# SHI-Labs/Self-Similarity-Grouping

Measured on AMD Instinct MI355X. Metric: images/s embed + s/iter for NxN rerank+DBSCAN, N=16k, 1/2/4/8 GPU, higher is better.
Workload: dtype f32 (embed: split-half operands hi+lo on fp16 MFMA, fp32 accumulate, 6e-8 max error vs the fp32 reference features) / exact int64 via int8 MFMA digits + f64 + f16 (distance, re-rank: half semantics, bit-exact)

## Files before the change

include/ssg_hip.h:

```cpp
#ifndef SSG_HIP_H
#define SSG_HIP_H

#include <stddef.h>
#include <stdint.h>

#ifdef __cplusplus
extern "C" {
#endif

typedef struct ihipStream_t* ssg_stream_t;

#define SSG_OK 0
#define SSG_ERR_INVALID (-1)
#define SSG_ERR_HIP (-2)
#define SSG_ERR_OVERFLOW (-3)
#define SSG_ERR_NAN (-4)

const char* ssg_last_error(void);
int ssg_version(void);
uint16_t ssg_double_to_half_bits(double d);

int ssg_range_stats_f32(const float* a, int rows_a, const float* b, int rows_b, int d, float* out4, ssg_stream_t stream);
int ssg_row_norms_f64(const float* x, int n, int d, int round_to_half, double* norms, ssg_stream_t stream);
int ssg_sqdist_self_f16(const float* x, const double* norms, int N, int d, int row0, int nrows, int memory_save, uint16_t* D, uint32_t* rowmax,
// ... 96 lines not shown
                      void* ws, size_t ws_bytes, int64_t* labels, ssg_stream_t stream);

int ssg_conv2d_nhwc_f32(const float* in, const float* w, const float* bias, const float* res, float* out, int B, int H, int W, int Cin,
                        int Cout, int KH, int KW, int stride, int pad, int relu, ssg_stream_t stream);
int ssg_conv1x1_dual_nhwc_f32(const float* in, const float* in2, const float* w, const float* bias, float* out, int B, int H, int W, int Cin,
                              int H2, int W2, int Cin2, int stride2, int Cout, int relu, ssg_stream_t stream);
#define SSG_CONV_IN_SPLIT 1
#define SSG_CONV_OUT_SPLIT 2
int ssg_conv2d_nhwc_x(const void* in, const void* w, const float* bias, const void* res, void* out, int B, int H, int W, int Cin,
                      int Cout, int KH, int KW, int stride, int pad, int relu, int flags, float acc_scale, const float* ch_scale,
                      int32_t* overflow, ssg_stream_t stream);
int ssg_conv1x1_dual_nhwc_x(const void* in, const void* in2, const void* w, const float* bias, void* out, int B, int H, int W, int Cin,
                            int H2, int W2, int Cin2, int stride2, int Cout, int relu, int flags, float acc_scale, const float* ch_scale,
                            int32_t* overflow, ssg_stream_t stream);
#define SSG_CONV_W_TILED 4
int ssg_conv_weights_tile_supported(int Cout, int Kpad);
int ssg_conv_weights_tile(const void* w, int Cout, int Kpad, void* wt, ssg_stream_t stream);
int ssg_conv2d_nhwc_xt(const void* in, const void* w, const void* wt, const float* bias, const void* res, void* out, int B, int H, int W, int Cin,
                       int Cout, int KH, int KW, int stride, int pad, int relu, int flags, float acc_scale, const float* ch_scale,
                       int32_t* overflow, ssg_stream_t stream);
int ssg_conv1x1_dual_nhwc_xt(const void* in, const void* in2, const void* w, const void* wt, const float* bias, void* out, int B, int H, int W, int Cin,
                             int H2, int W2, int Cin2, int stride2, int Cout, int relu, int flags, float acc_scale, const float* ch_scale,
                             int32_t* overflow, ssg_stream_t stream);
int ssg_conv_pair_supported(int K1, int C, int N2);
int ssg_conv_pair_nhwc_x(const void* y2, const void* w3, const float* b3, const float* cs3, const void* res, void* out,
                         const void* w1n, const float* b1n, const float* cs1n, void* y1n, int M, int K1, int C, int N2,
                         int32_t* overflow, ssg_stream_t stream);
int ssg_bottleneck_supported(int H, int W, int CIN, int C, int MID);
int ssg_bottleneck_nhwc_x(const void* x, const void* w1, const float* b1, const float* cs1, const void* w2, const float* b2, const float* cs2,
                          const void* w3, const float* b3, const float* cs3, void* out, int B, int H, int W, int C, int MID,
                          int32_t* overflow, ssg_stream_t stream);
int ssg_bottleneck_ds_nhwc_x(const void* x, const void* w1, const float* b1, const float* cs1, const void* w2, const float* b2, const float* cs2,
                             const void* w3cat, const float* b3, const float* cs3, void* out, int B, int H, int W, int CIN, int C, int MID,
                             int32_t* overflow, ssg_stream_t stream);
int ssg_basicblock_supported(int H, int W, int C);
int ssg_basicblock_nhwc_x(const void* x, const void* w1, const float* b1, const float* cs1, const void* w2, const float* b2, const float* cs2,
                          void* out, int B, int H, int W, int C, int32_t* overflow, ssg_stream_t stream);
int ssg_stem_pool_supported(int H, int W);
int ssg_stem_pool_nchw_x(const float* images, int flip, const void* w, const float* bias, const float* ch_scale, void* out, int B, int H, int W,
                         int32_t* overflow, ssg_stream_t stream);
int ssg_nchw_to_nhwc4_h4l4(const float* in, void* out, int B, int H, int W, int flip, ssg_stream_t stream);
int ssg_maxpool3x3s2_h8l8(const void* in, void* out, int B, int H, int W, int C, ssg_stream_t stream);
int ssg_gap_stripes_h8l8(const void* in, float* out, int B, int H, int W, int C, int num_split, ssg_stream_t stream);
int ssg_h8l8_encode(const float* in, void* out, int64_t n, float scale, ssg_stream_t stream);
int ssg_h8l8_decode(const void* in, float* out, int64_t n, float scale, ssg_stream_t stream);
int ssg_pairwise_sqdist_f32(const float* x, const float* y, int m, int n, int d, int self_form, float* ws, float* out, ssg_stream_t stream);
// ... 186 lines not shown
```

self-similarity-grouping_amd/csrc/conv.hip:

```cpp
#include "ssg_common.h"
#include <cstdlib>
#include <type_traits>

namespace ssg {

typedef float v16f __attribute__((ext_vector_type(16)));
typedef unsigned int v4u __attribute__((ext_vector_type(4)));
typedef _Float16 v8h __attribute__((ext_vector_type(8)));

__device__ __forceinline__ unsigned pack_h2(_Float16 a, _Float16 b) {
  return (unsigned)__builtin_bit_cast(unsigned short, a) | ((unsigned)__builtin_bit_cast(unsigned short, b) << 16);
}
__device__ __forceinline__ float unpack_lo(unsigned u) { return (float)__builtin_bit_cast(_Float16, (unsigned short)(u & 0xffffu)); }
__device__ __forceinline__ float unpack_hi(unsigned u) { return (float)__builtin_bit_cast(_Float16, (unsigned short)(u >> 16)); }
__device__ __forceinline__ void split_encode4(const float4 v, uint2& hi, uint2& lo) {
  const _Float16 h0 = (_Float16)v.x, h1 = (_Float16)v.y, h2 = (_Float16)v.z, h3 = (_Float16)v.w;
  hi = make_uint2(pack_h2(h0, h1), pack_h2(h2, h3));
  lo = make_uint2(pack_h2((_Float16)(v.x - (float)h0), (_Float16)(v.y - (float)h1)), pack_h2((_Float16)(v.z - (float)h2), (_Float16)(v.w - (float)h3)));
}
__device__ __forceinline__ bool split_hi_nonfinite(const uint2 hi) {
  const unsigned a = hi.x & 0x7fff7fffu, b = hi.y & 0x7fff7fffu;
  return (a & 0xffffu) >= 0x7c00u || (a >> 16) >= 0x7c00u || (b & 0xffffu) >= 0x7c00u || (b >> 16) >= 0x7c00u;
}
__device__ __forceinline__ float4 split_decode4(const uint2 hi, const uint2 lo) {
  return make_float4(unpack_lo(hi.x) + unpack_lo(lo.x), unpack_hi(hi.x) + unpack_hi(lo.x), unpack_lo(hi.y) + unpack_lo(lo.y), unpack_hi(hi.y) + unpack_hi(lo.y));
}

struct ConvParams {
  const float* in; const float* w; const float* bias; const float* res = nullptr; float* out;
  int B, H, W, Cin, OH, OW, Cout, KH, KW, stride, pad, relu;
  int M, Kpad;
  unsigned in_bytes;
  const float* in2 = nullptr; int H2 = 0, W2 = 0, Cin2 = 0, stride2 = 1, nk1; unsigned in2_bytes = 0;
  const float* rowterm = nullptr; int epi = 0;
  float* tilemin = nullptr; int tmin_ld = 0;
  int out_split = 0, res_split = 0; float acc_scale = 1.f;
  const float* cscale = nullptr;
  int* overflow = nullptr;
  const float* wt = nullptr;
  unsigned long long* prof = nullptr;
};
#ifdef SSG_DMA_PROF
#define SSG_DMA_STAMP(I_) { if (p.prof && threadIdx.x == 0) p.prof[(size_t)blockIdx.x * 8 + (I_)] = __builtin_readcyclecounter(); }
#else
#define SSG_DMA_STAMP(I_)
#endif

constexpr int CLD32 = 36;

__device__ __forceinline__ int conv_xcd_remap(int b, int nwg) {
  const int nx = 8, q = nwg / nx, r = nwg % nx, x = b % nx, s = b / nx;
  return (x < r ? x * (q + 1) : r * (q + 1) + (x - r) * q) + s;
}

template <int MT, int NT> struct SplitFrags { v8h ah[MT], al[MT], bh[NT], bl[NT]; };

typedef float v4f __attribute__((ext_vector_type(4)));
template <int MT, int NT, int CLD, bool TAP4>
__device__ __forceinline__ void split_load_frags(const float* Arow, const float* Brow, const int kofs, SplitFrags<MT, NT>& f) {
#pragma unroll
  for (int i = 0; i < MT; i++) {
    const float* q = Arow + i * 32 * CLD + kofs;
    if (TAP4) {
// ... 360 lines not shown
          v.x += r4.x; v.y += r4.y; v.z += r4.z; v.w += r4.w;
        }
        if (p.relu) { v.x = v.x > 0.f ? v.x : 0.f; v.y = v.y > 0.f ? v.y : 0.f; v.z = v.z > 0.f ? v.z : 0.f; v.w = v.w > 0.f ? v.w : 0.f; }
        if (p.out_split) {
          uint2 hp, lp;
          split_encode4(v, hp, lp);
          if (p.overflow && split_hi_nonfinite(hp)) *p.overflow = 1;
          const uint2 send = h ? hp : lp;
          const uint2 recv = make_uint2((unsigned)__shfl_xor((int)send.x, 32, 64), (unsigned)__shfl_xor((int)send.y, 32, 64));
          const uint4 st = h ? make_uint4(recv.x, recv.y, lp.x, lp.y) : make_uint4(hp.x, hp.y, recv.x, recv.y);
#ifdef SSG_IGEMM_NT_STORE
          if (m < p.M) { const v4u sv_ = {st.x, st.y, st.z, st.w}; __builtin_nontemporal_store(sv_, reinterpret_cast<v4u*>(outp + (int64_t)m * p.Cout + col)); }
#else
          if (m < p.M) *reinterpret_cast<uint4*>(outp + (int64_t)m * p.Cout + col) = st;
#endif
        } else if (m < p.M) *reinterpret_cast<float4*>(outp + (int64_t)m * p.Cout + col) = v;
      }
    }
  }
}

#define SSG_LDSP(ptr_) ((__attribute__((address_space(3))) void*)(ptr_))

template <int BM, int BN, bool DUAL = false, int LINE = 0>
__global__ __launch_bounds__((BM / 64) * (BN / 64) * 64, BM == 256 ? 1 : (BN == 256 ? 4 : 3)) void conv_dma_kernel(ConvParams p) {
  static_assert((BM == 128 && (BN == 128 || BN == 256)) || (BM == 256 && BN == 256), "128 x 128, 128 x 256 or 256 x 256 tiles");
  static_assert(LINE == 0 || LINE == 1, "k-tile order or line order");
  constexpr int NS = BM == 256 ? 4 : 3;
  constexpr int WM = 64, WN = 64, MT = WM / 32, NT = 2, CBK = 16;
  constexpr int WCOLS = BN / WN, NW = (BM / WM) * WCOLS;
  constexpr int ABLK = BM / 16 / NW, WBLK = BN / 16 / NW;
  constexpr int STAGE_BYTES = (BM + BN) * 64;
  __shared__ __attribute__((aligned(1024))) unsigned char st0[STAGE_BYTES];
  __shared__ __attribute__((aligned(1024))) unsigned char st1[STAGE_BYTES];
  __shared__ __attribute__((aligned(1024))) unsigned char st2[STAGE_BYTES];
  __shared__ __attribute__((aligned(1024))) unsigned char st3[NS == 4 ? STAGE_BYTES : 1024];
  const int tiles_n = p.Cout / BN, tiles_m = (p.M + BM - 1) / BM;
  const int tile = conv_xcd_remap((int)blockIdx.x, tiles_m * tiles_n);
  const int tm = tile / tiles_n, tn = tile % tiles_n;
  const int tid = (int)threadIdx.x, lane = tid & 63, wave = __builtin_amdgcn_readfirstlane(tid >> 6);
  SSG_DMA_STAMP(0)
  const int wm = wave / WCOLS, wn = wave % WCOLS, l32 = lane & 31, h = lane >> 5;

  const int drow = lane >> 2, pc = lane & 3;
  const int lc4 = (pc ^ ((drow >> 2) & 3)) * 4;
  const int nkA = DUAL ? p.nk1 * 2 : 0x7fffffff;
  int ab0, ah0, aw0, ab1 = -1, ah1 = 0, aw1 = 0, abase0 = 0, abase1 = 0;
  unsigned a2b0 = 0x80000000u, a2b1 = 0x80000000u;
#define SSG_ROW(J)                                                                                                   \
  {                                                                                                                  \
// ... 166 lines not shown
    if constexpr (NS == 4) { if (nk - nfull == 3) { asm volatile("s_waitcnt vmcnt(0) lgkmcnt(0)\n\ts_barrier" ::: "memory"); SSG_LAST(st2) } }
  }
#undef SSG_READS
#undef SSG_G1
#undef SSG_G2
#undef SSG_G3
#undef SSG_STEP
#undef SSG_LAST
  SSG_DMA_STAMP(2)
  __syncthreads();
  SSG_DMA_STAMP(3)
#undef SSG_DMA_NEXT
#undef SSG_DMA_A
#undef SSG_DMA_PAIR
#undef SSG_DMA_A2
#undef SSG_DMA_W
#pragma unroll
  for (int i = 0; i < MT; i++)
#pragma unroll
    for (int j = 0; j < NT; j++)
#pragma unroll
      for (int r = 0; r < 16; r++) acc[i][j][r] *= p.acc_scale;

  if (p.epi == 3) {
#pragma unroll
    for (int i = 0; i < MT; i++) {
      const int m = tm * BM + wm * WM + i * 32 + l32;
      const float rt = p.rowterm[m < p.M ? m : 0];
#pragma unroll
      for (int j = 0; j < NT; j++) {
        float gq[4];
#pragma unroll
        for (int q = 0; q < 4; q++) {
          const float4 bias = *reinterpret_cast<const float4*>(p.bias + tn * BN + wn * WN + j * 32 + 8 * q + 4 * h);
          float mn = fminf(fminf((rt + bias.x) - 2.f * acc[i][j][4 * q], (rt + bias.y) - 2.f * acc[i][j][4 * q + 1]),
                           fminf((rt + bias.z) - 2.f * acc[i][j][4 * q + 2], (rt + bias.w) - 2.f * acc[i][j][4 * q + 3]));
          gq[q] = fminf(mn, __shfl_xor(mn, 32, 64));
        }
        if (h == 0 && m < p.M)
          *reinterpret_cast<float4*>(p.tilemin + (int64_t)m * p.tmin_ld + (tn * BN + wn * WN + j * 32) / 8) = make_float4(gq[0], gq[1], gq[2], gq[3]);
      }
    }
    return;
  }
  constexpr int EP = 36, CPR = 8, RPI = 8, ITS = 4;
  constexpr int PPS = STAGE_BYTES / (32 * EP * 4) < 6 ? STAGE_BYTES / (32 * EP * 4) : 6;
  static_assert(PPS * 32 * EP * 4 <= STAGE_BYTES && 3 * PPS >= NW, "epilogue patches fit in the stage arrays");
  float* patch = reinterpret_cast<float*>(wave < PPS ? st0 : (wave < 2 * PPS ? st1 : st2)) + (wave % PPS) * (32 * EP);
  const int chunk = lane % CPR, prow = lane / CPR, odd = lane & 1;
  const float* __restrict__ resp = p.res;
  float* __restrict__ outp = p.out;
#ifndef SSG_DMA_RES_AUX
#define SSG_DMA_RES_AUX 2
#endif
#ifndef SSG_DMA_OUT_AUX_RES
#define SSG_DMA_OUT_AUX_RES 2
#endif
#ifndef SSG_DMA_OUT_AUX
#define SSG_DMA_OUT_AUX 0
#endif
  if (p.out_split && p.relu && p.cscale != nullptr && (resp == nullptr || p.res_split) &&
      ((int64_t)p.M + BM) * p.Cout * 4 < (int64_t)0xffffffff) {
    constexpr int NP = MT * NT;
    unsigned ovf = 0u;
    const unsigned tbytes = (unsigned)((int64_t)p.M * p.Cout * 4), rowb = (unsigned)p.Cout * 4u;
    const __amdgpu_buffer_rsrc_t out_rsrc = __builtin_amdgcn_make_buffer_rsrc(outp, 0, tbytes, 0x00020000);
    const __amdgpu_buffer_rsrc_t res_rsrc = __builtin_amdgcn_make_buffer_rsrc(const_cast<float*>(resp ? resp : outp), 0, resp ? tbytes : 0u, 0x00020000);
    const unsigned lane_off = (unsigned)prow * rowb + (unsigned)chunk * 16u;
    const unsigned ubase = (unsigned)(tm * BM + wm * WM) * rowb + (unsigned)(tn * BN + wn * WN) * 4u;
    auto poff = [&](const int n, const int it) { return ubase + (unsigned)((n % MT) * 32 + it * RPI) * rowb + (unsigned)(n / MT) * 128u + lane_off; };
    auto run = [&](auto RES_) {
      constexpr bool RES = decltype(RES_)::value;
      v4u rr[ITS];
      v4f bias = *reinterpret_cast<const v4f*>(p.bias + tn * BN + wn * WN + chunk * 4), cs = *reinterpret_cast<const v4f*>(p.cscale + tn * BN + wn * WN + chunk * 4);
      v4f bias_n = bias, cs_n = cs;
      if constexpr (RES) {
#pragma unroll
        for (int it = 0; it < ITS; it++) rr[it] = __builtin_amdgcn_raw_buffer_load_b128(res_rsrc, poff(0, it), 0, SSG_DMA_RES_AUX);
      }
#pragma unroll
      for (int n = 0; n < NP; n++) {
        const int j = n / MT, i = n % MT;
        if (n % MT == MT - 1 && j + 1 < NT) {
          bias_n = *reinterpret_cast<const v4f*>(p.bias + tn * BN + wn * WN + (j + 1) * 32 + chunk * 4);
          cs_n = *reinterpret_cast<const v4f*>(p.cscale + tn * BN + wn * WN + (j + 1) * 32 + chunk * 4);
        }
#pragma unroll
        for (int q = 0; q < 4; q++)
          *reinterpret_cast<float4*>(patch + l32 * EP + 8 * q + 4 * h) = make_float4(acc[i][j][4 * q], acc[i][j][4 * q + 1], acc[i][j][4 * q + 2], acc[i][j][4 * q + 3]);
        __builtin_amdgcn_fence(__ATOMIC_ACQ_REL, "wavefront");
#pragma unroll
        for (int it = 0; it < ITS; it++) {
          float4 v = *reinterpret_cast<const float4*>(patch + (it * RPI + prow) * EP + chunk * 4);
          v.x = v.x * cs[0] + bias[0]; v.y = v.y * cs[1] + bias[1]; v.z = v.z * cs[2] + bias[2]; v.w = v.w * cs[3] + bias[3];
          if constexpr (RES) {
            const unsigned a0 = rr[it][0], a1 = rr[it][1], a2 = rr[it][2], a3 = rr[it][3];
            if (n + 1 < NP) rr[it] = __builtin_amdgcn_raw_buffer_load_b128(res_rsrc, poff(n + 1, it), 0, SSG_DMA_RES_AUX);
            const unsigned g0 = lane_xor1(odd ? a0 : a2), g1 = lane_xor1(odd ? a1 : a3);
            const float4 r4 = split_decode4(make_uint2(odd ? g0 : a0, odd ? g1 : a1), make_uint2(odd ? a2 : g0, odd ? a3 : g1));
            v.x += r4.x; v.y += r4.y; v.z += r4.z; v.w += r4.w;
          }
          v.x = v.x > 0.f ? v.x : 0.f; v.y = v.y > 0.f ? v.y : 0.f; v.z = v.z > 0.f ? v.z : 0.f; v.w = v.w > 0.f ? v.w : 0.f;
          uint2 hp, lp;
          split_encode4(v, hp, lp);
          ovf |= ((hp.x & 0x7c007c00u) + 0x04000400u) | ((hp.y & 0x7c007c00u) + 0x04000400u);
          const unsigned rx = lane_xor1(odd ? hp.x : lp.x), ry = lane_xor1(odd ? hp.y : lp.y);
          const v4u stv = {odd ? rx : hp.x, odd ? ry : hp.y, odd ? lp.x : rx, odd ? lp.y : ry};
          __builtin_amdgcn_raw_buffer_store_b128(stv, out_rsrc, poff(n, it), 0, RES ? SSG_DMA_OUT_AUX_RES : SSG_DMA_OUT_AUX);
        }
        __builtin_amdgcn_fence(__ATOMIC_ACQ_REL, "wavefront");
        if (n % MT == MT - 1) { bias = bias_n; cs = cs_n; }
      }
    };
    if (resp) run(std::true_type{}); else run(std::false_type{});
    if ((ovf & 0x80008000u) && p.overflow) *p.overflow = 1;
    SSG_DMA_STAMP(4)
    return;
  }
#pragma unroll
  for (int i = 0; i < MT; i++) {
    const int mbase = tm * BM + wm * WM + i * 32;
#pragma unroll
    for (int j = 0; j < NT; j++) {
      const int col = tn * BN + wn * WN + j * 32 + chunk * 4;
      const float4 bias = *reinterpret_cast<const float4*>(p.bias + col);
      const float4 cs = p.cscale ? *reinterpret_cast<const float4*>(p.cscale + col) : make_float4(1.f, 1.f, 1.f, 1.f);
      float4 rr[ITS];
      if (resp) {
#pragma unroll
        for (int it = 0; it < ITS; it++) {
          const int m = mbase + it * RPI + prow;
          rr[it] = *reinterpret_cast<const float4*>(resp + (int64_t)(m < p.M ? m : 0) * p.Cout + col);
        }
      }
#pragma unroll
      for (int q = 0; q < 4; q++)
        *reinterpret_cast<float4*>(patch + l32 * EP + 8 * q + 4 * h) = make_float4(acc[i][j][4 * q], acc[i][j][4 * q + 1], acc[i][j][4 * q + 2], acc[i][j][4 * q + 3]);
// ... 214 lines not shown
  else if (cin4 || !split) { wide = false; bn64 = p.Cout % 128 != 0; }
  else {
    wide = k.wide_mintiles > 0 && p.Cout % 256 == 0 && p.Kpad >= 128 && rows128 * (p.Cout / 256) >= k.wide_mintiles;
    bn64 = p.Cout % 128 != 0 || rows128 * (p.Cout / 128) < k.bn64_maxtiles;
  }
  if (wide) r.BN = 256; else if (bn64) r.BN = 64;
  bool dma;
  if (wide) {
    dma = (k.dma & 1) && (p.epi == 0 || p.epi == 3) && (int64_t)p.Cout * p.Kpad * 4 < 0x7fffffffLL;
    const int tiles_tall = ((p.M + 255) / 256) * (p.Cout / 256);
    if (dma && k.tall_mintiles > 0 && p.epi == 0 && tiles_tall >= k.tall_mintiles && (dual ? k.tall_dual != 0 : (!p.res || k.tall_res))) r.BM = 256;
  } else {
    dma = split && !cin4 && r.BN == 128 && (k.dma & 2) && p.epi == 0 && !dual;
    if (!dma) r.BK = split ? (cin4 ? 16 : 32) : (dual ? 32 : 16);
  }
  if (!dma) return r;
  r.family = CONV_DMA; r.BK = 16;
  if (p.epi != 0 || ((p.Kpad / 16) & 1) || (p.Cin % 32) || (dual && (p.Cin2 % 32))) r.line = 0;
  else if (k.line >= 0) r.line = k.line;
  else r.line = (r.BM == 256 && dual) ? 0 : 1;
  return r;
}

static ConvKnobs read_conv_knobs() {
  auto knob_int = [](const char* name, int dflt) { const char* e = getenv(name); return e ? atoi(e) : dflt; };
  ConvKnobs k;
  k.dma = knob_int("SSG_CONV_DMA", k.dma);
  if (const char* e = getenv("SSG_CONV_LINE")) k.line = atoi(e) == 1 ? 1 : 0;
  k.wide_mintiles = knob_int("SSG_SPLIT_WIDE_MINTILES", k.wide_mintiles);
  k.bn64_maxtiles = knob_int("SSG_SPLIT_BN64_MAXTILES", k.bn64_maxtiles);
  k.tall_mintiles = knob_int("SSG_CONV_TALL_MINTILES", k.tall_mintiles);
  k.tall_res = knob_int("SSG_CONV_TALL_RES", k.tall_res);
  k.tall_dual = knob_int("SSG_CONV_TALL_DUAL", k.tall_dual);
  return k;
}
static const ConvKnobs& conv_knobs() { static const ConvKnobs k = read_conv_knobs(); return k; }

template <int BM, int BN, bool DUAL>
static int launch_conv_dma(const ConvParams& p, int line, hipStream_t stream) {
  const int tiles = ((p.M + BM - 1) / BM) * (p.Cout / BN);
  if (line) hipLaunchKernelGGL((conv_dma_kernel<BM, BN, DUAL, 1>), dim3(tiles), dim3((BM / 64) * (BN / 64) * 64), 0, stream, p);
  else hipLaunchKernelGGL((conv_dma_kernel<BM, BN, DUAL, 0>), dim3(tiles), dim3((BM / 64) * (BN / 64) * 64), 0, stream, p);
  return ssg_check_hip(hipGetLastError(), "conv_dma_kernel");
}

template <int BN, int WN>
static int launch_conv_igemm(const ConvParams& p, const ConvRoute& r, bool split, bool cin4, hipStream_t stream) {
  if (cin4) return split ? launch_conv_bk<128, BN, 64, WN, true, 16, true>(p, stream) : launch_conv_bk<128, BN, 64, WN, true, 16, false>(p, stream);
  if (split) return launch_conv_bk<128, BN, 64, WN, false, 32, true>(p, stream);
  return r.BK == 32 ? launch_conv_bk<128, BN, 64, WN, false, 32, false>(p, stream) : launch_conv_bk<128, BN, 64, WN, false, 16, false>(p, stream);
}

static int launch_conv(const ConvParams& p, bool split, bool cin4, hipStream_t stream) {
  const ConvRoute r = conv_route(p, split, cin4, conv_knobs());
  if (r.family == CONV_DMA) {
    if (r.BM == 256) return r.dual ? launch_conv_dma<256, 256, true>(p, r.line, stream) : launch_conv_dma<256, 256, false>(p, r.line, stream);
    if (r.BN == 256) return r.dual ? launch_conv_dma<128, 256, true>(p, r.line, stream) : launch_conv_dma<128, 256, false>(p, r.line, stream);
    return launch_conv_dma<128, 128, false>(p, r.line, stream);
  }
  if (r.BN == 256) return launch_conv_bk<128, 256, 64, 64, false, 32, true>(p, stream);
  return r.BN == 128 ? launch_conv_igemm<128, 64>(p, r, split, cin4, stream) : launch_conv_igemm<64, 32>(p, r, split, cin4, stream);
}

static ConvParams conv_gemm_params(const float* x, const float* y, const float* bias, float* out, int m, int n, int d) {
  ConvParams p;
  p.in = x; p.w = y; p.bias = bias; p.out = out;
  p.B = p.M = m; p.H = p.W = p.OH = p.OW = 1; p.Cin = p.Kpad = d; p.Cout = n; p.KH = p.KW = 1; p.stride = 1; p.pad = 0; p.relu = 0;
  p.nk1 = d / 16; p.in_bytes = (unsigned)((int64_t)m * d * 4);
  return p;
}

extern "C" int ssg_conv_weights_tile_supported(int Cout, int Kpad) { return Cout > 0 && Kpad > 0 && Cout % 128 == 0 && Kpad % 16 == 0; }

extern "C" int ssg_conv_weights_tile(const void* w, int Cout, int Kpad, void* wt, hipStream_t stream) {
  if (!ssg_conv_weights_tile_supported(Cout, Kpad)) return 0;
  if (!w || !wt || (((uintptr_t)w | (uintptr_t)wt) & 15)) { ssg_set_error("ssg_conv_weights_tile: w and wt must be given and 16-byte aligned"); return SSG_ERR_INVALID; }
  const int64_t nslots = (int64_t)Cout * Kpad / 4;
// ... 15 lines not shown
extern "C" int ssg_conv2d_nhwc_xt(const void* in, const void* w, const void* wt, const float* bias, const void* res, void* out, int B, int H, int W,
                                  int Cin, int Cout, int KH, int KW, int stride, int pad, int relu, int flags, float acc_scale, const float* ch_scale,
                                  int32_t* overflow, hipStream_t stream) {
  ConvParams p;
  p.cscale = ch_scale; p.overflow = overflow;
  p.in = (const float*)in; p.w = (const float*)w; p.bias = bias; p.res = (const float*)res; p.out = (float*)out;
  p.B = B; p.H = H; p.W = W; p.Cin = Cin; p.Cout = Cout; p.KH = KH; p.KW = KW; p.stride = stride; p.pad = pad; p.relu = relu;
  p.OH = (H + 2 * pad - KH) / stride + 1; p.OW = (W + 2 * pad - KW) / stride + 1;
  const int64_t M = (int64_t)B * p.OH * p.OW;
  const bool split = (flags & 1) != 0;
  if (B <= 0 || M <= 0 || M > 0x7fffffff || (Cout % 64) || !((Cin % 32) == 0 || Cin == 4) || stride < 1) {
    ssg_set_error("ssg_conv2d_nhwc: unsupported shape B=%d H=%d W=%d Cin=%d Cout=%d k=%dx%d s=%d p=%d flags=%d", B, H, W, Cin, Cout, KH, KW, stride, pad, flags);
    return SSG_ERR_INVALID;
  }
  p.M = (int)M;
  const int64_t in_bytes = (int64_t)B * H * W * Cin * 4;
  if (in_bytes > 0x7fffffffLL) { ssg_set_error("ssg_conv2d_nhwc: input tensor of %lld bytes exceeds the 2 GiB buffer-resource range of this kernel; use a smaller batch", (long long)in_bytes); return SSG_ERR_INVALID; }
  p.in_bytes = (unsigned)in_bytes;
  p.out_split = (flags & 2) ? 1 : 0; p.res_split = p.out_split; p.acc_scale = acc_scale;
  const bool cin4 = (Cin == 4);
  p.Kpad = cin4 ? 32 * ((KH * KW + 7) / 8) : KH * KW * Cin;
  p.nk1 = p.Kpad / 16;
  { int rc; p.wt = (const float*)conv_tiled_weights("ssg_conv2d_nhwc_xt", w, wt, flags, Cout, p.Kpad, &rc); if (rc) return rc; }
  return launch_conv(p, split, cin4, stream);
}

extern "C" int ssg_conv2d_nhwc_x(const void* in, const void* w, const float* bias, const void* res, void* out, int B, int H, int W,
                                 int Cin, int Cout, int KH, int KW, int stride, int pad, int relu, int flags, float acc_scale, const float* ch_scale,
                                 int32_t* overflow, hipStream_t stream) {
  return ssg_conv2d_nhwc_xt(in, w, nullptr, bias, res, out, B, H, W, Cin, Cout, KH, KW, stride, pad, relu, flags, acc_scale, ch_scale, overflow, stream);
}

extern "C" int ssg_conv2d_nhwc_f32(const float* in, const float* w, const float* bias, const float* res, float* out, int B, int H, int W,
                                   int Cin, int Cout, int KH, int KW, int stride, int pad, int relu, hipStream_t stream) {
  return ssg_conv2d_nhwc_x(in, w, bias, res, out, B, H, W, Cin, Cout, KH, KW, stride, pad, relu, 0, 1.f, nullptr, nullptr, stream);
}

extern "C" int ssg_conv1x1_dual_nhwc_xt(const void* in, const void* in2, const void* w, const void* wt, const float* bias, void* out, int B, int H, int W,
                                        int Cin, int H2, int W2, int Cin2, int stride2, int Cout, int relu, int flags, float acc_scale, const float* ch_scale,
                                        int32_t* overflow, hipStream_t stream) {
  ConvParams p;
  p.cscale = ch_scale; p.overflow = overflow;
  p.in = (const float*)in; p.w = (const float*)w; p.bias = bias; p.out = (float*)out;
  p.B = B; p.H = H; p.W = W; p.Cin = Cin; p.Cout = Cout; p.KH = 1; p.KW = 1; p.stride = 1; p.pad = 0; p.relu = relu;
  p.OH = H; p.OW = W;
  const int64_t M = (int64_t)B * H * W;
  const int64_t in_bytes = M * Cin * 4, in2_bytes = (int64_t)B * H2 * W2 * Cin2 * 4;
  if (B <= 0 || M > 0x7fffffff || (Cout % 64) || (Cin % 32) || (Cin2 % 32) || stride2 < 1 || (H - 1) * stride2 >= H2 || (W - 1) * stride2 >= W2 ||
// ... 132 lines not shown
```

self-similarity-grouping_amd/resnet.py:

```python
from collections import OrderedDict

import math
import os

import torch

from . import _lib
from ._lib import check, ptr, stream

_LAYERS = {18: (2, 2, 2, 2), 34: (3, 4, 6, 3), 50: (3, 4, 6, 3), 101: (3, 4, 23, 3), 152: (3, 8, 36, 3)}
_BASIC = (18, 34)
_BN_EPS = 1e-5
_DEC_CLUSTERS, _DEC_DIM, _DEC_KEY = 32, 2048, "assignment.cluster_centers"
_FUSED_BASICBLOCK_DEFAULT = "1"


def _expansion(depth):
    return 1 if depth in _BASIC else 4


def _arch(depth):
    blocks = []
    inplanes = 64
    exp = _expansion(depth)
# ... 39 lines not shown
        conv(p + ".conv1", pl, ip, 1); bn(p + ".bn1", pl)
        conv(p + ".conv2", pl, pl, 3); bn(p + ".bn2", pl)
        conv(p + ".conv3", pl * 4, pl, 1); bn(p + ".bn3", pl * 4)
        if blk["down"]:
            conv(p + ".downsample.0", pl * 4, ip, 1); bn(p + ".downsample.1", pl * 4)
    sd["base.fc.weight"] = torch.randn(1000, width, generator=g) * 0.01
    sd["base.fc.bias"] = torch.zeros(1000)
    if num_features > 0:
        sd["feat.weight"] = torch.randn(num_features, width, generator=g) * 0.001
        sd["feat_bn.weight"] = torch.ones(num_features); sd["feat_bn.bias"] = torch.zeros(num_features)
        sd["feat_bn.running_mean"] = torch.zeros(num_features); sd["feat_bn.running_var"] = torch.ones(num_features)
        sd["feat_bn.num_batches_tracked"] = torch.zeros((), dtype=torch.long)
    if cluster:
        bound = math.sqrt(6.0 / (_DEC_CLUSTERS + _DEC_DIM))
        sd[_DEC_KEY] = (torch.rand(_DEC_CLUSTERS, _DEC_DIM, generator=g) * 2.0 - 1.0) * bound
    return sd


class _FoldedConv:
    __slots__ = ("w", "bias", "cin", "cout", "k", "stride", "pad", "split", "acc_scale", "cscale", "wt")


_IN_SPLIT, _OUT_SPLIT, _W_TILED = 1, 2, 4


def _attach_tiled(f):
    f.wt = None
    cout, kp = f.w.shape
    if not f.split or f.cin == 4 or f.w.device.type != "cuda":
        return f
    L = _lib.lib()
    if not L.ssg_conv_weights_tile_supported(cout, kp):
        return f
    both = torch.empty((2, cout, kp), dtype=torch.float32, device=f.w.device)
    both[0].copy_(f.w)
    rc = L.ssg_conv_weights_tile(ptr(both[0]), cout, kp, ptr(both[1]), stream())
    if rc != 1:
        check(rc if rc < 0 else -2, "ssg_conv_weights_tile")
    f.w, f.wt = both[0], both[1]
    return f


def _h8l8(v):
    rows, K = v.shape
    hi = v.half()
    lo = (v - hi.float()).half()
# ... 99 lines not shown

class ResNet:

    def __init__(self, depth=50, checkpoint=None, pretrained=True, num_features=2048, dropout=0.1, num_classes=0, num_split=1,
                 mode='Dissimilarity', cluster=False, seed=1, precision=None):
        if depth not in _LAYERS:
            raise KeyError("Unsupported depth:", depth)
        if num_classes > 0:
            raise NotImplementedError("num_classes > 0 (dropout + classifier head, resnet.py:118-120) is a training-only path; "
                                      "the grouping path uses num_classes=0 (selftraining.py:121-123)")
        if num_features > 0 and num_features % 64:
            raise ValueError("num_features must be a multiple of 64")
        self.depth, self.num_features, self.dropout, self.num_classes = depth, num_features, dropout, num_classes
        self.out_planes = 512 * _expansion(depth)
        self.num_split, self.cluster, self.pretrained, self.training = num_split, cluster, pretrained, False
        self.precision = precision or os.environ.get("SSG_EMBED_PRECISION", "split")
        if self.precision not in ("split", "f32"):
            raise ValueError("precision must be 'split' or 'f32'")
        self.device = torch.device("cpu")
        self._sd = synthetic_state_dict(seed, depth, num_features, cluster=bool(cluster))
        self._folded = None
        self._twin = None
        self.tiled_weights = os.environ.get("SSG_CONV_WT", "1") != "0"
        self.flip_streams = True
        self._weights = "synthetic"
        if checkpoint:
            self.load_state_dict(torch.load(checkpoint, map_location="cpu"), strict=False)
        elif pretrained:
            import warnings
            warnings.warn("ssg_amd ResNet(pretrained=True): no ImageNet weights are available offline; the backbone holds seeded "
                          "synthetic weights until load_state_dict()/checkpoint= supplies real ones", stacklevel=2)

    def state_dict(self):
        return OrderedDict((k, v.clone() if v.device.type == "cpu" else v.cpu()) for k, v in self._sd.items())

    def load_state_dict(self, state_dict, strict=True):
        state_dict, missing, unexpected = self._match_keys(state_dict, strict)
        for k, v in state_dict.items():
            if k in self._sd:
                if tuple(v.shape) != tuple(self._sd[k].shape):
                    raise RuntimeError("size mismatch for %s: %r vs %r" % (k, tuple(v.shape), tuple(self._sd[k].shape)))
                self._sd[k] = v.detach().to("cpu").clone()
        self._invalidate()
        self._report_missing("load_state_dict", missing)
        return missing, unexpected

# ... 103 lines not shown
        fold = self._fold_one
        net = dict(stem=fold("base.conv1", "base.bn1", 2, 3, sp), blocks=[], split=sp)
        for blk in _arch(self.depth):
            p = blk["prefix"]
            if blk["kind"] == "basic":
                net["blocks"].append(dict(
                    kind="basic",
                    c1=fold(p + ".conv1", p + ".bn1", blk["stride"], 1, sp),
                    c2=fold(p + ".conv2", p + ".bn2", 1, 1, sp),
                    ds=fold(p + ".downsample.0", p + ".downsample.1", blk["stride"], 0, sp) if blk["down"] else None))
                continue
            if blk["down"]:
                c3, ds = self._fold_dual(p, blk["stride"], sp)
            else:
                c3, ds = fold(p + ".conv3", p + ".bn3", 1, 0, sp), None
            net["blocks"].append(dict(
                c1=fold(p + ".conv1", p + ".bn1", 1, 0, sp),
                c2=fold(p + ".conv2", p + ".bn2", blk["stride"], 1, sp),
                c3=c3, ds=ds))
        self._folded = net
        return net

    @staticmethod
    def _conv(L, x, f, res=None, relu=True, out_split=False, ovf=None, tiled=False):
        B, H, W, _ = x.shape
        OH = (H + 2 * f.pad - f.k) // f.stride + 1; OW = (W + 2 * f.pad - f.k) // f.stride + 1
        out = torch.empty((B, OH, OW, f.cout), dtype=torch.float32, device=x.device)
        flags = (_IN_SPLIT if f.split else 0) | (_OUT_SPLIT if out_split else 0) | (_W_TILED if tiled and f.wt is not None else 0)
        check(L.ssg_conv2d_nhwc_x(ptr(x), ptr(f.w), ptr(f.bias), ptr(res), ptr(out), B, H, W, f.cin, f.cout, f.k, f.k, f.stride, f.pad,
                                  1 if relu else 0, flags, f.acc_scale, ptr(getattr(f, "cscale", None)), ptr(ovf), stream()), "ssg_conv2d_nhwc_x")
        return out

    @staticmethod
    def _conv_dual(L, o, x, c3, ds, out_split=False, ovf=None, tiled=False):
        B, H, W, _ = o.shape
        _, H2, W2, _ = x.shape
        out = torch.empty((B, H, W, c3.cout), dtype=torch.float32, device=o.device)
        flags = (_IN_SPLIT if ds.split else 0) | (_OUT_SPLIT if out_split else 0) | (_W_TILED if tiled and ds.wt is not None else 0)
        check(L.ssg_conv1x1_dual_nhwc_x(ptr(o), ptr(x), ptr(ds.w), ptr(ds.bias), ptr(out), B, H, W, c3.cin, H2, W2, ds.cin, ds.stride, c3.cout, 1,
                                        flags, ds.acc_scale, ptr(getattr(ds, "cscale", None)), ptr(ovf), stream()), "ssg_conv1x1_dual_nhwc_x")
        return out

    @staticmethod
    def _bottleneck(L, y, blk, ovf=None):
        B, H, W, CIN = y.shape
        c1, c2, c3, ds = blk["c1"], blk["c2"], blk["c3"], blk["ds"]
        if os.environ.get("SSG_FUSED_BOTTLENECK", "1") == "0" or c2.stride != 1 or (ds is not None and ds.stride != 1):
            return None
        if not L.ssg_bottleneck_supported(H, W, CIN, c3.cout, c1.cout):
            return None
        out = torch.empty((B, H, W, c3.cout), dtype=torch.float32, device=y.device)
        if ds is None:
            check(L.ssg_bottleneck_nhwc_x(ptr(y), ptr(c1.w), ptr(c1.bias), ptr(c1.cscale), ptr(c2.w), ptr(c2.bias), ptr(c2.cscale),
                                          ptr(c3.w), ptr(c3.bias), ptr(c3.cscale), ptr(out), B, H, W, CIN, c1.cout, ptr(ovf), stream()),
                  "ssg_bottleneck_nhwc_x")
        else:
            check(L.ssg_bottleneck_ds_nhwc_x(ptr(y), ptr(c1.w), ptr(c1.bias), ptr(c1.cscale), ptr(c2.w), ptr(c2.bias), ptr(c2.cscale),
                                             ptr(ds.w), ptr(ds.bias), ptr(ds.cscale), ptr(out), B, H, W, CIN, c3.cout, c1.cout, ptr(ovf), stream()),
                  "ssg_bottleneck_ds_nhwc_x")
        return out

    @staticmethod
    def _basicblock(L, y, blk, ovf=None):
        B, H, W, C = y.shape
        c1, c2 = blk["c1"], blk["c2"]
        if os.environ.get("SSG_FUSED_BASICBLOCK", _FUSED_BASICBLOCK_DEFAULT) == "0" or c1.stride != 1 or blk["ds"] is not None or c1.cout != C:
            return None
        if not L.ssg_basicblock_supported(H, W, C):
            return None
        out = torch.empty((B, H, W, C), dtype=torch.float32, device=y.device)
        check(L.ssg_basicblock_nhwc_x(ptr(y), ptr(c1.w), ptr(c1.bias), ptr(c1.cscale), ptr(c2.w), ptr(c2.bias), ptr(c2.cscale), ptr(out),
                                      B, H, W, C, ptr(ovf), stream()), "ssg_basicblock_nhwc_x")
        return out

    def _fmap(self, x, flip=False, hooks=None):
        L = _lib.lib()
        net = self._prepare()
        sp = net["split"]
        tw = bool(getattr(self, "tiled_weights", True))
        x = x.to(self.device, torch.float32).contiguous()
        B, C, H, W = x.shape
        if C != 3:
            raise ValueError("expected RGB images [B,3,H,W]")
        ovf = self._overflow_flag() if sp else None
        if sp and os.environ.get("SSG_FUSED_STEM", "1") != "0" and L.ssg_stem_pool_supported(H, W):
            st = net["stem"]
            y = torch.empty((B, H // 4, W // 4, 64), dtype=torch.float32, device=self.device)
            check(L.ssg_stem_pool_nchw_x(ptr(x), 1 if flip else 0, ptr(st.w), ptr(st.bias), ptr(st.cscale), ptr(y), B, H, W, ptr(ovf), stream()),
                  "ssg_stem_pool_nchw_x")
        else:
            x4 = torch.empty((B, H, W, 4), dtype=torch.float32, device=self.device)
            if sp:
                check(L.ssg_nchw_to_nhwc4_h4l4(ptr(x), ptr(x4), B, H, W, 1 if flip else 0, stream()), "ssg_nchw_to_nhwc4_h4l4")
            else:
                check(L.ssg_nchw_to_nhwc4(ptr(x), ptr(x4), B, H, W, 1 if flip else 0, stream()), "ssg_nchw_to_nhwc4")
            y = self._conv(L, x4, net["stem"], out_split=sp, ovf=ovf)
            _, H2, W2, _ = y.shape
            p = torch.empty((B, (H2 + 1) // 2, (W2 + 1) // 2, 64), dtype=torch.float32, device=self.device)
# ... 13 lines not shown
                    y = fused
                    continue
                o = self._conv(L, y, blk["c1"], out_split=sp, ovf=ovf, tiled=tw)
                r = y if blk["ds"] is None else self._conv(L, y, blk["ds"], relu=False, out_split=sp, ovf=ovf, tiled=tw)
                y = self._conv(L, o, blk["c2"], res=r, relu=True, out_split=sp, ovf=ovf, tiled=tw)
                continue
            if sp:
                fused = self._bottleneck(L, y, blk, ovf)
                if fused is not None:
                    y = fused
                    continue
            o = o1_next if o1_next is not None else self._conv(L, y, blk["c1"], out_split=sp, ovf=ovf, tiled=tw)
            o1_next = None
            o = self._conv(L, o, blk["c2"], out_split=sp, ovf=ovf, tiled=tw)
            if blk["ds"] is not None:
                y = self._conv_dual(L, o, y, blk["c3"], blk["ds"], out_split=sp, ovf=ovf, tiled=tw)
                continue
            nxt = blocks[bi + 1]["c1"] if bi + 1 < len(blocks) else None
            Bo, Ho, Wo, _ = o.shape
            if (pair and nxt is not None and nxt.k == 1 and nxt.stride == 1 and nxt.cin == blk["c3"].cout and Bo * Ho * Wo >= 128 * 256
                    and L.ssg_conv_pair_supported(blk["c3"].cin, blk["c3"].cout, nxt.cout)):
                y, o1_next = self._conv_pair(L, o, blk["c3"], y, nxt, ovf)
            else:
                y = self._conv(L, o, blk["c3"], res=y, relu=True, out_split=sp, ovf=ovf, tiled=tw)
        return y, sp

    @staticmethod
    def _conv_pair(L, o, c3, res, c1n, ovf=None):
        B, H, W, _ = o.shape
        out = torch.empty((B, H, W, c3.cout), dtype=torch.float32, device=o.device)
        y1n = torch.empty((B, H, W, c1n.cout), dtype=torch.float32, device=o.device)
        check(L.ssg_conv_pair_nhwc_x(ptr(o), ptr(c3.w), ptr(c3.bias), ptr(c3.cscale), ptr(res), ptr(out), ptr(c1n.w), ptr(c1n.bias), ptr(c1n.cscale),
                                     ptr(y1n), B * H * W, c3.cin, c3.cout, c1n.cout, ptr(ovf), stream()), "ssg_conv_pair_nhwc_x")
        return out, y1n

    def _side_streams(self):
        st = getattr(self, "_streams", None)
        if st is None or st[0].device != self.device:
            prio = -1 if os.environ.get("SSG_FLIP_PRIO", "0") == "1" else 0
            st = self._streams = (torch.cuda.Stream(self.device, priority=prio), torch.cuda.Stream(self.device))
        return st

    def _overflow_flag(self):
        if getattr(self, "_ovf", None) is None or self._ovf.device != self.device:
            self._ovf = torch.zeros(1, dtype=torch.int32, device=self.device)
        return self._ovf

# ... 5 lines not shown
            self._ovf.zero_()
        return hit

    def _f32_twin(self):
        if getattr(self, "_twin", None) is None:
            import warnings
            warnings.warn("ssg_amd ResNet: an activation left the half range of the split-half path (|v| >= 65520); this batch and any "
                          "later one that overflows is recomputed with precision='f32'", stacklevel=3)
            t = ResNet.__new__(ResNet)
            t.__dict__.update({k: v for k, v in self.__dict__.items() if k not in ("_folded", "_ovf", "_twin")})
            t.precision, t._folded, t._ovf, t._twin = "f32", None, None, None
            self._twin = t
        return self._twin

    def feature_map(self, x, flip=False):
        y, sp = self._fmap(x, flip)
        if sp:
            if self._overflowed():
                return self._f32_twin().feature_map(x, flip)
            out = torch.empty_like(y)
            check(_lib.lib().ssg_h8l8_decode(ptr(y), ptr(out), y.numel(), 1.0, stream()), "ssg_h8l8_decode")
            return out
        return y

    def pooled(self, fmap, split=False):
        L = _lib.lib()
        B, h, w, C = fmap.shape
        S = self.num_split if self.num_split > 1 else 1
        if S > h:
            raise _lib.SSGError("num_split = %d stripes on a layer4 map of %d rows (input height too small): no such feature" % (S, h))
        nsets = S + 1 if S > 1 else 1
        out = torch.empty((nsets, B, C), dtype=torch.float32, device=fmap.device)
        if split:
            check(L.ssg_gap_stripes_h8l8(ptr(fmap), ptr(out), B, h, w, C, S, stream()), "ssg_gap_stripes_h8l8")
        else:
            check(L.ssg_gap_stripes(ptr(fmap), ptr(out), B, h, w, C, S, stream()), "ssg_gap_stripes")
        return out

    def _x2(self, gap):
        if self.num_features <= 0:
            return None
        net = self._prepare()
        if "feat" not in net:
            keys = _bn_keys("feat", "feat_bn")
            if _use_device_fold(self._sd, keys):
                src = [self._sd[k] for k in keys]
# ... 4 lines not shown
                f = _fold({"c.weight": sd["feat.weight"].view(self.num_features, self.out_planes, 1, 1), "b.weight": sd["feat_bn.weight"],
                           "b.bias": sd["feat_bn.bias"], "b.running_mean": sd["feat_bn.running_mean"], "b.running_var": sd["feat_bn.running_var"]},
                          "c", "b", 1, 0, self.device)
            net["feat"] = f
        B = gap.shape[0]
        out = self._conv(_lib.lib(), gap.reshape(B, 1, 1, self.out_planes).contiguous(), net["feat"], relu=True)
        return out.reshape(B, self.num_features)

    def _x3(self, x1):
        from . import dce
        net = self._prepare()
        if "centers" not in net:
            net["centers"] = self._sd[_DEC_KEY].to(self.device, torch.float32).contiguous()
        return dce.soft_assignment(x1, net["centers"], 1.0)

    def __call__(self, x, for_eval=False):
        if self.cluster and self.num_split > 1 and not for_eval:
            raise ValueError("cluster=True with num_split=%d and for_eval=False: the reference assigns the concatenated [B, %d] features to "
                             "%d-wide cluster centres, a shape mismatch (reid/models/resnet.py:129)"
                             % (self.num_split, (self.num_split + 1) * self.out_planes, _DEC_DIM))
        if self.cluster and self.num_split <= 1 and self.out_planes != _DEC_DIM:
            raise ValueError("cluster=True on a %d-wide backbone (resnet%d): the reference assigns [B, %d] features to %d-wide cluster "
                             "centres, a shape mismatch (reid/models/resnet.py:129-131)" % (self.out_planes, self.depth, self.out_planes, _DEC_DIM))
        sets = self.pooled(*self._fmap(x))
        if self._overflowed():
            return self._f32_twin()(x, for_eval)
        x2 = self._x2(sets[0])
        if self.num_split > 1:
            x1 = [sets[s] for s in range(sets.shape[0])]
            if for_eval:
                return torch.cat(x1, dim=1), x2
            return x1, x2
        if self.cluster:
            return sets[0], x2, self._x3(sets[0])
        return sets[0], x2

    forward = __call__

    def embed_with_flip(self, x, for_eval=False, check_overflow=True):
        L = _lib.lib()
        x = x.to(self.device, torch.float32)
        if self.flip_streams and self.precision == "split" and os.environ.get("SSG_FLIP_STREAMS", "1") != "0":
            cur = torch.cuda.current_stream(self.device)
            ready = torch.cuda.Event(); ready.record(cur)
            ab = []
            for st, flip in zip(self._side_streams(), (False, True)):
                st.wait_event(ready)
                with torch.cuda.stream(st):
                    r = self.pooled(*self._fmap(x, flip=flip))
                r.record_stream(cur)
                ab.append(r)
            for st in self._side_streams():
                cur.wait_stream(st)
            a, b = ab
        else:
            a = self.pooled(*self._fmap(x, flip=False))
            b = self.pooled(*self._fmap(x, flip=True))
        if check_overflow and self._overflowed():
            return self._f32_twin().embed_with_flip(x, for_eval)
        nsets, B, C = a.shape
        if for_eval or nsets == 1:
            a = a.permute(1, 0, 2).reshape(B, nsets * C).contiguous(); b = b.permute(1, 0, 2).reshape(B, nsets * C).contiguous()
            out = torch.empty_like(a)
            check(L.ssg_flip_sum_l2norm(ptr(a), ptr(b), ptr(out), B, nsets * C, stream()), "ssg_flip_sum_l2norm")
            return out
        out = torch.empty_like(a)
        check(L.ssg_flip_sum_l2norm(ptr(a), ptr(b), ptr(out), nsets * B, C, stream()), "ssg_flip_sum_l2norm")
        return out


def resnet18(**kwargs):
    return ResNet(18, **kwargs)


def resnet34(**kwargs):
    return ResNet(34, **kwargs)


def resnet50(**kwargs):
    return ResNet(50, **kwargs)
# ... 22 lines not shown
```

Before: 28980.

## Fuse global and stripe average pooling into last bottleneck conv epilogue

Adds a POOL instance of the 128x256 LDS-DMA conv kernel that pools the final block's output in its epilogue. Tiles are decoded into LDS and averaged per image, both globally and per stripe, instead of writing the split-half feature map and running a separate pooling kernel. This removes a full feature-map write and read plus one launch per flip pass. In exchange it adds a templated kernel variant, a capability check and a Python routing path, and only applies when OH*OW == 32.

After: 29100, median of 4. No clear change (+0.4%).

```diff
diff --git a/include/ssg_hip.h b/include/ssg_hip.h
--- a/include/ssg_hip.h
+++ b/include/ssg_hip.h
@@ -142,6 +142,9 @@
 int ssg_conv1x1_dual_nhwc_xt(const void* in, const void* in2, const void* w, const void* wt, const float* bias, void* out, int B, int H, int W, int Cin,
                              int H2, int W2, int Cin2, int stride2, int Cout, int relu, int flags, float acc_scale, const float* ch_scale,
                              int32_t* overflow, ssg_stream_t stream);
+#define SSG_CONV_OUT_POOL 256
+#define SSG_CONV_POOL_STRIPES(flags) (((flags) >> 16) & 255)
+int ssg_conv_pool_supported(int B, int OH, int OW, int Cin, int Cout, int S);
 int ssg_conv_pair_supported(int K1, int C, int N2);
 int ssg_conv_pair_nhwc_x(const void* y2, const void* w3, const float* b3, const float* cs3, const void* res, void* out,
                          const void* w1n, const float* b1n, const float* cs1n, void* y1n, int M, int K1, int C, int N2,
diff --git a/self-similarity-grouping_amd/csrc/conv.hip b/self-similarity-grouping_amd/csrc/conv.hip
--- a/self-similarity-grouping_amd/csrc/conv.hip
+++ b/self-similarity-grouping_amd/csrc/conv.hip
@@ -39,6 +39,7 @@
   int* overflow = nullptr;
   const float* wt = nullptr;
   unsigned long long* prof = nullptr;
+  int pool_stripes = 0;
 };
 #ifdef SSG_DMA_PROF
 #define SSG_DMA_STAMP(I_) { if (p.prof && threadIdx.x == 0) p.prof[(size_t)blockIdx.x * 8 + (I_)] = __builtin_readcyclecounter(); }
@@ -445,10 +446,11 @@
 
 #define SSG_LDSP(ptr_) ((__attribute__((address_space(3))) void*)(ptr_))
 
-template <int BM, int BN, bool DUAL = false, int LINE = 0>
+template <int BM, int BN, bool DUAL = false, int LINE = 0, bool POOL = false>
 __global__ __launch_bounds__((BM / 64) * (BN / 64) * 64, BM == 256 ? 1 : (BN == 256 ? 4 : 3)) void conv_dma_kernel(ConvParams p) {
   static_assert((BM == 128 && (BN == 128 || BN == 256)) || (BM == 256 && BN == 256), "128 x 128, 128 x 256 or 256 x 256 tiles");
   static_assert(LINE == 0 || LINE == 1, "k-tile order or line order");
+  static_assert(!POOL || (BM == 128 && BN == 256 && !DUAL), "the pooling epilogue exists for the 128 x 256 instance");
   constexpr int NS = BM == 256 ? 4 : 3;
   constexpr int WM = 64, WN = 64, MT = WM / 32, NT = 2, CBK = 16;
   constexpr int WCOLS = BN / WN, NW = (BM / WM) * WCOLS;
@@ -661,7 +663,7 @@
 #pragma unroll
       for (int r = 0; r < 16; r++) acc[i][j][r] *= p.acc_scale;
 
-  if (p.epi == 3) {
+  if (!POOL && p.epi == 3) {
 #pragma unroll
     for (int i = 0; i < MT; i++) {
       const int m = tm * BM + wm * WM + i * 32 + l32;
@@ -698,8 +700,8 @@
 #ifndef SSG_DMA_OUT_AUX
 #define SSG_DMA_OUT_AUX 0
 #endif
-  if (p.out_split && p.relu && p.cscale != nullptr && (resp == nullptr || p.res_split) &&
-      ((int64_t)p.M + BM) * p.Cout * 4 < (int64_t)0xffffffff) {
+  if (POOL || (p.out_split && p.relu && p.cscale != nullptr && (resp == nullptr || p.res_split) &&
+      ((int64_t)p.M + BM) * p.Cout * 4 < (int64_t)0xffffffff)) {
     constexpr int NP = MT * NT;
     unsigned ovf = 0u;
     const unsigned tbytes = (unsigned)((int64_t)p.M * p.Cout * 4), rowb = (unsigned)p.Cout * 4u;
@@ -743,15 +745,41 @@
           uint2 hp, lp;
           split_encode4(v, hp, lp);
           ovf |= ((hp.x & 0x7c007c00u) + 0x04000400u) | ((hp.y & 0x7c007c00u) + 0x04000400u);
-          const unsigned rx = lane_xor1(odd ? hp.x : lp.x), ry = lane_xor1(odd ? hp.y : lp.y);
-          const v4u stv = {odd ? rx : hp.x, odd ? ry : hp.y, odd ? lp.x : rx, odd ? lp.y : ry};
-          __builtin_amdgcn_raw_buffer_store_b128(stv, out_rsrc, poff(n, it), 0, RES ? SSG_DMA_OUT_AUX_RES : SSG_DMA_OUT_AUX);
+          if constexpr (POOL) {
+            *reinterpret_cast<float4*>(patch + (it * RPI + prow) * EP + chunk * 4) = split_decode4(hp, lp);
+          } else {
+            const unsigned rx = lane_xor1(odd ? hp.x : lp.x), ry = lane_xor1(odd ? hp.y : lp.y);
+            const v4u stv = {odd ? rx : hp.x, odd ? ry : hp.y, odd ? lp.x : rx, odd ? lp.y : ry};
+            __builtin_amdgcn_raw_buffer_store_b128(stv, out_rsrc, poff(n, it), 0, RES ? SSG_DMA_OUT_AUX_RES : SSG_DMA_OUT_AUX);
+          }
         }
         __builtin_amdgcn_fence(__ATOMIC_ACQ_REL, "wavefront");
+        if constexpr (POOL) {
+          const int img = (tm * BM + wm * WM + i * 32) >> 5, ch = tn * BN + wn * WN + j * 32 + l32;
+          const int S = p.pool_stripes;
+          const int seg = h ? (S > 1 ? (p.OH / S) * p.OW : 0) : 32, last = h && S > 1 ? S : 0;
+          int set = h, cnt = 0;
+          float a = 0.f;
+#pragma unroll 1
+          for (int r0 = 0; r0 < 32; r0 += 8) {
+            float pv[8];
+#pragma unroll
+            for (int u = 0; u < 8; u++) pv[u] = patch[(r0 + u) * EP + l32];
+#pragma unroll
+            for (int u = 0; u < 8; u++) {
+              a += pv[u];
+              if (++cnt == seg) {
+                if (set <= last && img < p.B) outp[((int64_t)set * p.B + img) * p.Cout + ch] = a / (float)seg;
+                a = 0.f; cnt = 0; set++;
+              }
+            }
+          }
+          __builtin_amdgcn_fence(__ATOMIC_ACQ_REL, "wavefront");
+        }
         if (n % MT == MT - 1) { bias = bias_n; cs = cs_n; }
       }
     };
-    if (resp) run(std::true_type{}); else run(std::false_type{});
+    if (POOL || resp) run(std::true_type{}); else run(std::false_type{});
     if ((ovf & 0x80008000u) && p.overflow) *p.overflow = 1;
     SSG_DMA_STAMP(4)
     return;
@@ -1012,6 +1040,20 @@
   return r;
 }
 
+static bool conv_pool_takes(const ConvParams& p, const ConvRoute& r, int S) {
+  return r.family == CONV_DMA && r.BM == 128 && r.BN == 256 && !r.dual && p.epi == 0 && p.res != nullptr && p.res_split && p.out_split && p.relu &&
+         p.cscale != nullptr && p.OH * p.OW == 32 && S >= 1 && S <= p.OH && ((int64_t)p.M + 128) * p.Cout * 4 < (int64_t)0xffffffff;
+}
+static bool conv_pool_supported(int B, int OH, int OW, int Cin, int Cout, int S, const ConvKnobs& k) {
+  if (B <= 0 || OH <= 0 || OW <= 0 || Cin <= 0 || Cout <= 0 || (Cin % 32) || (Cout % 64) || S < 0 || S > 255 || (int64_t)B * OH * OW > 0x7fffffff) return false;
+  ConvParams p = {};
+  p.res = p.cscale = reinterpret_cast<const float*>(&p);
+  p.B = B; p.H = p.OH = OH; p.W = p.OW = OW; p.Cin = Cin; p.Cout = Cout; p.KH = p.KW = 1; p.stride = 1; p.relu = 1;
+  p.M = B * OH * OW; p.Kpad = Cin; p.nk1 = Cin / 16;
+  p.out_split = p.res_split = 1;
+  return conv_pool_takes(p, conv_route(p, true, false, k), S > 1 ? S : 1);
+}
+
 static ConvKnobs read_conv_knobs() {
   auto knob_int = [](const char* name, int dflt) { const char* e = getenv(name); return e ? atoi(e) : dflt; };
   ConvKnobs k;
@@ -1026,11 +1068,11 @@
 }
 static const ConvKnobs& conv_knobs() { static const ConvKnobs k = read_conv_knobs(); return k; }
 
-template <int BM, int BN, bool DUAL>
+template <int BM, int BN, bool DUAL, bool POOL = false>
 static int launch_conv_dma(const ConvParams& p, int line, hipStream_t stream) {
   const int tiles = ((p.M + BM - 1) / BM) * (p.Cout / BN);
-  if (line) hipLaunchKernelGGL((conv_dma_kernel<BM, BN, DUAL, 1>), dim3(tiles), dim3((BM / 64) * (BN / 64) * 64), 0, stream, p);
-  else hipLaunchKernelGGL((conv_dma_kernel<BM, BN, DUAL, 0>), dim3(tiles), dim3((BM / 64) * (BN / 64) * 64), 0, stream, p);
+  if (line) hipLaunchKernelGGL((conv_dma_kernel<BM, BN, DUAL, 1, POOL>), dim3(tiles), dim3((BM / 64) * (BN / 64) * 64), 0, stream, p);
+  else hipLaunchKernelGGL((conv_dma_kernel<BM, BN, DUAL, 0, POOL>), dim3(tiles), dim3((BM / 64) * (BN / 64) * 64), 0, stream, p);
   return ssg_check_hip(hipGetLastError(), "conv_dma_kernel");
 }
 
@@ -1043,6 +1085,7 @@
 
 static int launch_conv(const ConvParams& p, bool split, bool cin4, hipStream_t stream) {
   const ConvRoute r = conv_route(p, split, cin4, conv_knobs());
+  if (p.pool_stripes) return launch_conv_dma<128, 256, false, true>(p, r.line, stream);
   if (r.family == CONV_DMA) {
     if (r.BM == 256) return r.dual ? launch_conv_dma<256, 256, true>(p, r.line, stream) : launch_conv_dma<256, 256, false>(p, r.line, stream);
     if (r.BN == 256) return r.dual ? launch_conv_dma<128, 256, true>(p, r.line, stream) : launch_conv_dma<128, 256, false>(p, r.line, stream);
@@ -1104,8 +1147,20 @@
   p.Kpad = cin4 ? 32 * ((KH * KW + 7) / 8) : KH * KW * Cin;
   p.nk1 = p.Kpad / 16;
   { int rc; p.wt = (const float*)conv_tiled_weights("ssg_conv2d_nhwc_xt", w, wt, flags, Cout, p.Kpad, &rc); if (rc) return rc; }
+  if (flags & 256) {
+    const int S = (flags >> 16) & 255;
+    p.pool_stripes = S > 1 ? S : 1;
+    if (!conv_pool_takes(p, conv_route(p, split, cin4, conv_knobs()), p.pool_stripes)) {
+      ssg_set_error("ssg_conv2d_nhwc: SSG_CONV_OUT_POOL needs a launch of the 128x256 LDS-DMA kernel with a split-half residual and output, ReLU, channel "
+                    "scales, OH*OW == 32 and stripes <= OH -- ask ssg_conv_pool_supported first (B=%d OH=%d OW=%d Cin=%d Cout=%d k=%dx%d res=%d flags=%d)",
+                    B, p.OH, p.OW, Cin, Cout, KH, KW, res != nullptr, flags);
+      return SSG_ERR_INVALID;
+    }
+  }
   return launch_conv(p, split, cin4, stream);
 }
+
+extern "C" int ssg_conv_pool_supported(int B, int OH, int OW, int Cin, int Cout, int S) { return conv_pool_supported(B, OH, OW, Cin, Cout, S, conv_knobs()) ? 1 : 0; }
 
 extern "C" int ssg_conv2d_nhwc_x(const void* in, const void* w, const float* bias, const void* res, void* out, int B, int H, int W,
                                  int Cin, int Cout, int KH, int KW, int stride, int pad, int relu, int flags, float acc_scale, const float* ch_scale,
diff --git a/self-similarity-grouping_amd/resnet.py b/self-similarity-grouping_amd/resnet.py
--- a/self-similarity-grouping_amd/resnet.py
+++ b/self-similarity-grouping_amd/resnet.py
@@ -85,6 +85,7 @@
 
 
 _IN_SPLIT, _OUT_SPLIT, _W_TILED = 1, 2, 4
+_OUT_POOL = 256
 
 
 def _attach_tiled(f):
@@ -230,6 +231,7 @@
         self._folded = None
         self._twin = None
         self.tiled_weights = os.environ.get("SSG_CONV_WT", "1") != "0"
+        self.fused_pool = os.environ.get("SSG_FUSED_POOL", "1") != "0"
         self.flip_streams = True
         self._weights = "synthetic"
         if checkpoint:
@@ -379,11 +381,13 @@
         return net
 
     @staticmethod
-    def _conv(L, x, f, res=None, relu=True, out_split=False, ovf=None, tiled=False):
+    def _conv(L, x, f, res=None, relu=True, out_split=False, ovf=None, tiled=False, pool=0):
         B, H, W, _ = x.shape
         OH = (H + 2 * f.pad - f.k) // f.stride + 1; OW = (W + 2 * f.pad - f.k) // f.stride + 1
-        out = torch.empty((B, OH, OW, f.cout), dtype=torch.float32, device=x.device)
+        out = torch.empty((B, OH, OW, f.cout) if not pool else (pool + 1 if pool > 1 else 1, B, f.cout), dtype=torch.float32, device=x.device)
         flags = (_IN_SPLIT if f.split else 0) | (_OUT_SPLIT if out_split else 0) | (_W_TILED if tiled and f.wt is not None else 0)
+        if pool:
+            flags |= _OUT_POOL | (pool << 16)
         check(L.ssg_conv2d_nhwc_x(ptr(x), ptr(f.w), ptr(f.bias), ptr(res), ptr(out), B, H, W, f.cin, f.cout, f.k, f.k, f.stride, f.pad,
                                   1 if relu else 0, flags, f.acc_scale, ptr(getattr(f, "cscale", None)), ptr(ovf), stream()), "ssg_conv2d_nhwc_x")
         return out
@@ -430,7 +434,7 @@
                                       B, H, W, C, ptr(ovf), stream()), "ssg_basicblock_nhwc_x")
         return out
 
-    def _fmap(self, x, flip=False, hooks=None):
+    def _fmap(self, x, flip=False, hooks=None, pool=False):
         L = _lib.lib()
         net = self._prepare()
         sp = net["split"]
@@ -490,7 +494,14 @@
                     and L.ssg_conv_pair_supported(blk["c3"].cin, blk["c3"].cout, nxt.cout)):
                 y, o1_next = self._conv_pair(L, o, blk["c3"], y, nxt, ovf)
             else:
-                y = self._conv(L, o, blk["c3"], res=y, relu=True, out_split=sp, ovf=ovf, tiled=tw)
+                S = 0
+                if pool and sp and bi == len(blocks) - 1:
+                    S = self.num_split if self.num_split > 1 else 1
+                    if not L.ssg_conv_pool_supported(Bo, Ho, Wo, blk["c3"].cin, blk["c3"].cout, S):
+                        S = 0
+                y = self._conv(L, o, blk["c3"], res=y, relu=True, out_split=sp, ovf=ovf, tiled=tw, pool=S)
+                if S:
+                    return y, None
         return y, sp
 
     @staticmethod
@@ -542,6 +553,10 @@
             check(_lib.lib().ssg_h8l8_decode(ptr(y), ptr(out), y.numel(), 1.0, stream()), "ssg_h8l8_decode")
             return out
         return y
+
+    def _sets(self, x, flip=False):
+        y, sp = self._fmap(x, flip=flip, pool=bool(getattr(self, "fused_pool", True)))
+        return y if sp is None else self.pooled(y, sp)
 
     def pooled(self, fmap, split=False):
         L = _lib.lib()
@@ -592,7 +607,7 @@
         if self.cluster and self.num_split <= 1 and self.out_planes != _DEC_DIM:
             raise ValueError("cluster=True on a %d-wide backbone (resnet%d): the reference assigns [B, %d] features to %d-wide cluster "
                              "centres, a shape mismatch (reid/models/resnet.py:129-131)" % (self.out_planes, self.depth, self.out_planes, _DEC_DIM))
-        sets = self.pooled(*self._fmap(x))
+        sets = self._sets(x)
         if self._overflowed():
             return self._f32_twin()(x, for_eval)
         x2 = self._x2(sets[0])
@@ -617,15 +632,15 @@
             for st, flip in zip(self._side_streams(), (False, True)):
                 st.wait_event(ready)
                 with torch.cuda.stream(st):
-                    r = self.pooled(*self._fmap(x, flip=flip))
+                    r = self._sets(x, flip=flip)
                 r.record_stream(cur)
                 ab.append(r)
             for st in self._side_streams():
                 cur.wait_stream(st)
             a, b = ab
         else:
-            a = self.pooled(*self._fmap(x, flip=False))
-            b = self.pooled(*self._fmap(x, flip=True))
+            a = self._sets(x, flip=False)
+            b = self._sets(x, flip=True)
         if check_overflow and self._overflowed():
             return self._f32_twin().embed_with_flip(x, for_eval)
         nsets, B, C = a.shape
```
